# MycroftAI/mycroft-precise

Measured on AMD Instinct MI355X. Metric: MFCC+GRU windows/sec (node); max concurrent real-time 16 kHz streams, higher is better.
Workload: dtype f32

## Files before the change

### include/precise_engine.h

```cpp
#ifndef PRECISE_ENGINE_H
#define PRECISE_ENGINE_H

#include <stddef.h>
#include <stdint.h>

#ifdef __cplusplus
extern "C" {
#endif

#define PE_ABI_VERSION 8

typedef enum pe_status {
    PE_OK = 0,
    PE_ERR_INVALID = 1,
    PE_ERR_HIP = 2,
    PE_ERR_UNSUPPORTED = 3,
    PE_ERR_NOMEM = 4,
    PE_ERR_EOF = 5
} pe_status;

typedef struct pe_params {
    int32_t sample_rate;
    int32_t window_samples;
    int32_t hop_samples;
// ... 92 lines not shown
int pe_decode_device(pe_engine* e, const float* raw_dev, double* conf_out_dev, unsigned char* fired_out_dev, void* hip_stream);
int pe_decode(pe_engine* e, const float* raw_host, double* conf_out_host, unsigned char* fired_out_host);

typedef struct pe_info {
    int32_t n_streams, n_features, n_mfcc, units, n_layers, ring_slots, carry_capacity;
    int32_t mfcc_precision, gru_precision;
    int64_t device_bytes;
} pe_info;
int pe_get_info(const pe_engine* e, pe_info* out);

int pe_get_stream_state(pe_engine* e, int32_t* q_out, uint32_t* computed_out, uint32_t* emitted_out);

int pe_set_renumber_at(pe_engine* e, uint32_t call_number);

int pe_set_fused(pe_engine* e, int32_t enabled);

int pe_set_input_projection(pe_engine* e, int32_t enabled);

int pe_set_gru_waves(pe_engine* e, int32_t waves_per_tile);

int pe_set_gru_tiling(pe_engine* e, int32_t tiling);
int pe_get_gru_tiling(const pe_engine* e);

int pe_set_timing(pe_engine* e, int32_t enabled);
int pe_get_last_timing(pe_engine* e, float* mfcc_ms, float* gru_ms);

#ifdef __cplusplus
}
#endif
#endif
```

### mycroft_precise_amd/_lib.py

```python
import ctypes as C
import importlib.util
import os
import weakref

import numpy as np

HERE = os.path.dirname(os.path.abspath(__file__))
LIB_PATH = os.environ.get('PE_LIB') or os.path.join(HERE, 'libprecise_engine.so')

PE_OK, PE_ERR_INVALID, PE_ERR_HIP, PE_ERR_UNSUPPORTED, PE_ERR_NOMEM, PE_ERR_EOF = range(6)
ABI_VERSION = 8


class PeParams(C.Structure):
    _fields_ = [(n, C.c_int32) for n in (
        'sample_rate', 'window_samples', 'hop_samples', 'n_fft', 'n_filt', 'n_mfcc', 'n_features',
        'use_delta', 'mfcc_precision', 'gru_precision', 'vectorizer', 'ring_precision')]


class PeGruLayer(C.Structure):
    _fields_ = [('n_in', C.c_int32), ('units', C.c_int32),
                ('kernel', C.POINTER(C.c_float)), ('recurrent_kernel', C.POINTER(C.c_float)),
                ('bias', C.POINTER(C.c_float))]

# ... 38 lines not shown
    'pe_get_vectors': (C.c_int, [C.c_void_p, C.c_void_p]),
    'pe_set_vectors': (C.c_int, [C.c_void_p, C.c_void_p]),
    'pe_run_device': (C.c_int, [C.c_void_p, C.c_void_p, C.c_void_p]),
    'pe_predict': (C.c_int, [C.c_void_p, C.c_void_p, C.c_int32, C.c_void_p]),
    'pe_predict_device': (C.c_int, [C.c_void_p, C.c_void_p, C.c_int32, C.c_void_p, C.c_void_p]),
    'pe_vectorize_raw': (C.c_int, [C.c_void_p, C.c_void_p, C.c_int64, C.c_void_p, C.c_int64,
                                   C.POINTER(C.c_int64)]),
    'pe_vectorize_mels': (C.c_int, [C.c_void_p, C.c_void_p, C.c_int64, C.c_void_p, C.c_int64,
                                   C.POINTER(C.c_int64)]),
    'pe_evaluate': (C.c_int, [C.c_void_p, C.c_void_p, C.c_int64, C.c_int32, C.c_void_p, C.c_int64,
                              C.POINTER(C.c_int64)]),
    'pe_set_decoder': (C.c_int, [C.c_void_p, C.c_void_p, C.c_int32, C.c_int32, C.c_int32, C.c_double]),
    'pe_set_trigger': (C.c_int, [C.c_void_p, C.c_int32, C.c_double, C.c_int32]),
    'pe_set_decoder_model': (C.c_int, [C.c_void_p, C.c_int32, C.c_void_p, C.c_int32, C.c_int32, C.c_int32, C.c_double]),
    'pe_set_trigger_model': (C.c_int, [C.c_void_p, C.c_int32, C.c_int32, C.c_double, C.c_int32]),
    'pe_decode_device': (C.c_int, [C.c_void_p, C.c_void_p, C.c_void_p, C.c_void_p, C.c_void_p]),
    'pe_decode': (C.c_int, [C.c_void_p, C.c_void_p, C.c_void_p, C.c_void_p]),
    'pe_get_info': (C.c_int, [C.c_void_p, C.POINTER(PeInfo)]),
    'pe_get_stream_state': (C.c_int, [C.c_void_p, C.c_void_p, C.c_void_p, C.c_void_p]),
    'pe_set_fused': (C.c_int, [C.c_void_p, C.c_int32]),
    'pe_set_gru_waves': (C.c_int, [C.c_void_p, C.c_int32]),
    'pe_set_gru_tiling': (C.c_int, [C.c_void_p, C.c_int32]),
    'pe_get_gru_tiling': (C.c_int, [C.c_void_p]),
    'pe_set_input_projection': (C.c_int, [C.c_void_p, C.c_int32]),
    'pe_set_timing': (C.c_int, [C.c_void_p, C.c_int32]),
    'pe_get_last_timing': (C.c_int, [C.c_void_p, C.POINTER(C.c_float), C.POINTER(C.c_float)]),
}

_lib = None


class HipLibraryMissing(ImportError):
    pass


def _preload_hip_runtime():
    if os.environ.get('PRECISE_AMD_HIP_RUNTIME', '') == 'system':
        return
    try:
        spec = importlib.util.find_spec('torch')
    except (ImportError, ValueError):
        spec = None
    if spec is None or not spec.origin:
        return
    cand = os.path.join(os.path.dirname(spec.origin), 'lib', 'libamdhip64.so')
    if os.path.exists(cand):
# ... 301 lines not shown

    def stream_state(self):
        q = np.empty(self.n_streams, dtype=np.int32)
        kc = np.empty(self.n_streams, dtype=np.uint32)
        ke = np.empty(self.n_streams, dtype=np.uint32)
        self._check(self._lib.pe_get_stream_state(self._h, q.ctypes.data, kc.ctypes.data, ke.ctypes.data))
        return q, kc, ke

    def set_fused(self, enabled: bool):
        self._check(self._lib.pe_set_fused(self._h, int(bool(enabled))))

    def set_input_projection(self, enabled: bool):
        self._check(self._lib.pe_set_input_projection(self._h, int(bool(enabled))))

    def set_gru_waves(self, waves: int):
        self._check(self._lib.pe_set_gru_waves(self._h, int(waves)))

    def set_gru_tiling(self, tiling: int):
        self._check(self._lib.pe_set_gru_tiling(self._h, int(tiling)))

    def gru_tiling(self) -> int:
        return int(self._lib.pe_get_gru_tiling(self._h))

    def set_timing(self, enabled: bool):
        self._check(self._lib.pe_set_timing(self._h, int(bool(enabled))))

    def last_timing(self):
        a, b = C.c_float(0), C.c_float(0)
        self._check(self._lib.pe_get_last_timing(self._h, C.byref(a), C.byref(b)))
        return a.value, b.value

    def close(self):
        if getattr(self, '_h', None) and self._h.value:
            if getattr(self, '_views', 0) > 0:
                self._close_pending = True
                try:
                    self._lib.pe_wait(self._h)
                except Exception:
                    pass
                return
            self._lib.pe_destroy(self._h)
            self._h = C.c_void_p()

    def __del__(self):
        try:
            self.close()
# ... 3 lines not shown
```

### mycroft_precise_amd/csrc/engine.hip

```cpp
#include "../../include/precise_engine.h"
#include "pe_common.h"
#include "gru_cw_pack.h"
#include "mfcc_general_device.h"

#include <algorithm>
#include <cmath>
#include <cstdarg>
#include <cstdio>
#include <cstdlib>
#include <cstring>
#include <string>
#include <vector>

using namespace pe;

namespace {

thread_local std::string g_global_error;

struct DeviceBuf {
    void* p = nullptr;
    size_t bytes = 0;
};

// ... 19 lines not shown
    int device = 0;
    int n_streams = 0, n_tiles = 0, n_padded = 0;
    int units = 0, n_in = 0, n_layers = 0;
    int ring_slots = 0;
    int mel_nnz = 0;
    std::string err;
    std::vector<void*> allocs;
    int64_t device_bytes = 0;
    StreamRec* rec = nullptr;
    int16_t* carry = nullptr;
    const int16_t* kept = nullptr; int kept_chunk = 0;
    const int16_t* call_head = nullptr; int call_head_chunk = 0; bool call_keep = false;
    uint32_t call_no = 1;
    uint32_t renumber_at = 0x7fff0000u;
    bool fused = true;
    int gru_waves = 0;
    bool general = false;
    int row_floats = kRowFloats;
    int carry_cap = kCarryCap;
    GeneralTables gtab{};
    int gru_tiling = -1;
    int n_cus = 256;
    float* ring = nullptr;
    float* proj_ring = nullptr;
    bool proj_ok = false, proj_on = false;
    std::vector<float> proj_w_host, proj_b_host;
    int max_updates = 1;
    uint32_t* ke_hist = nullptr;
    unsigned char* table_blob = nullptr;
    pe_wave::Layout table_layout{};
    int n_models = 1;
    std::vector<NetPack> nets;
    std::vector<DecState> dec;
    bool wide = false;
    int wide_kx4[2] = {1, 1};
    int32_t* activation = nullptr;
    DeviceBuf st_pcm, st_out, st_feats, st_mask, st_audio, st_mfcc, st_conf, st_fired, st_ids;
    std::vector<uint8_t> seen_ids;
    bool timing = false;
    hipEvent_t ev[3] = {nullptr, nullptr, nullptr};
    bool ev_valid = false, ev_has_gru = false;
    static constexpr int kAsyncDepth = 3;
    struct AsyncSlot {
        float* pin_out = nullptr; size_t pin_out_bytes = 0;
        DeviceBuf dev_in, dev_out;
        hipEvent_t copied = nullptr, done = nullptr;
// ... 605 lines not shown
}

ModelNet model_net(const NetPack& n, const GruArgs& a) {
    return ModelNet{n.wx, n.wxd, n.wr1, n.wr2, n.bias, n.wd, a.cw ? n.cw_blob : nullptr, n.wx_bf16, n.wr_bf16, n.wd_bf16,
                    a.b20 ? n.b20_blob : nullptr, a.x3 ? n.x3_blob : nullptr, n.dense_bias};
}
GruArgs with_model(const pe_engine* e, const GruArgs& a, int m) { return model_args(a, model_net(e->nets[m], a), 0, 0); }
ModelSet model_set(const pe_engine* e, const GruArgs& a) {
    ModelSet ms{};
    for (int m = 0; m < e->n_models; ++m) ms.net[m] = model_net(e->nets[m], a);
    return ms;
}

GruArgs gru_args(const pe_engine* e) {
    const NetPack& n0 = e->nets[0];
    GruArgs a{};
    a.n_streams = e->n_streams;
    a.n_features = e->prm.n_features;
    a.n_in = e->n_in;
    a.units = e->units;
    a.use_delta = e->prm.use_delta;
    a.ring = e->ring; a.ring_slots = e->ring_slots; a.ring_bf16 = e->prm.ring_precision;
    a.ids = nullptr; a.rec = e->rec; a.n_padded = (uint32_t)e->n_padded; a.ke_plain = nullptr;
    a.call = e->call_no + 1u;
    a.proj_ring = e->proj_on ? e->proj_ring : nullptr;
    a.predict_ke = 0;
    a.chunk = 0;
    a.window = emit_window(e->prm); a.hop = e->prm.hop_samples;
    a.frame_len = frame_len_of(e->prm);
    a.bf16 = e->prm.gru_precision == 1;
    a.b20 = e->gru_tiling == 0 ? nullptr : n0.b20_blob;
    a.feats = nullptr; a.out = nullptr; a.row_stride = 0;
    a.row_floats = e->row_floats;
    const bool x3_ok = n0.x3_blob && !a.bf16 && !e->wide && !a.proj_ring && e->row_floats == kRowFloats;
    const bool many_windows = e->max_updates > 1 && (long long)e->max_updates * e->n_tiles > 4LL * e->n_cus;
    a.x3 = x3_ok && (e->gru_tiling == 2 || (e->gru_tiling < 0 && (e->n_tiles > 4 * e->n_cus || many_windows))) ? n0.x3_blob : nullptr;
    const bool cw_ok = n0.cw_blob && e->row_floats == kRowFloats && !a.proj_ring && !a.bf16 && !a.x3 && !e->wide;
    const bool retile = cw_ok && (e->gru_tiling == 1 || (e->gru_tiling < 0 && e->n_tiles <= 2 * e->n_cus));
    const int auto_waves = retile ? (e->n_tiles <= 2 * e->n_cus ? 4 : 1) : (e->n_tiles <= e->n_cus ? 4 : 1);
    a.waves_per_tile = a.x3 ? 1 : e->gru_waves ? e->gru_waves : auto_waves;
    if (e->prm.use_delta && !retile) a.waves_per_tile = 1;
    if (e->row_floats != kRowFloats && !(gru_small_regs(e->units) == 5 && !e->prm.use_delta && a.waves_per_tile == 4))
        a.waves_per_tile = 1;
    a.cw = retile ? n0.cw_blob : nullptr;
    return with_model(e, a, 0);
}
// ... 95 lines not shown
    e->last_user_stream = static_cast<hipStream_t>(stream);
    e->user_dirty = true;
}

int check_chunk(pe_engine* e, const void* pcm, int chunk) {
    if (!e) return PE_ERR_INVALID;
    if (chunk == 0) return fail(e, PE_ERR_EOF, "empty chunk");
    if (chunk < 0 || !pcm) return fail(e, PE_ERR_INVALID, "bad pcm buffer / chunk_samples=%d", chunk);
    return PE_OK;
}

int flush_kept(pe_engine* e, hipStream_t s) {
    if (!e->kept) return PE_OK;
    PE_HIP(e, launch_materialize_carry(state_of(e, e->call_no + 1u), e->kept, e->kept_chunk, e->n_streams, s));
    e->kept = nullptr; e->kept_chunk = 0;
    return PE_OK;
}

bool keep_eligible(const pe_engine* e, const int16_t* pcm_dev, int chunk) {
    return !e->general && (chunk & 1) == 0 && (reinterpret_cast<uintptr_t>(pcm_dev) & 3u) == 0 && chunk >= frame_len_of(e->prm) - 1
        && chunk >= e->carry_cap - 1;
}

bool can_fuse(const pe_engine* e, int chunk) {
    if (!(e->fused && !e->general && !e->wide && e->table_layout.mel_pad == 10 && chunk <= emit_window(e->prm) - frame_len_of(e->prm))) return false;
    if (gru_args(e).x3) return false;
    if (e->prm.gru_precision == 0 && gru_small_regs(e->units) >= 6 && gru_args(e).waves_per_tile != 4) return false;
    if (e->prm.use_delta && e->prm.gru_precision == 0) {
        const GruArgs g = gru_args(e);
        if (g.cw && (g.waves_per_tile != 4 || e->ring_slots != kCwSlots || e->prm.n_features > kCwSlots)) return false;
    }
    return true;
}

int do_update(pe_engine* e, const int16_t* pcm_dev, int chunk, float* raw_out_dev, float* feats_out_dev,
              hipStream_t s, const int32_t* ids = nullptr, int n_active = 0, bool keep = false) {
    int rc;
    const bool t = e->timing;
    const bool keep_call = keep && !ids && keep_eligible(e, pcm_dev, chunk);
    if (keep_call && e->kept) {
        const char* a0 = reinterpret_cast<const char*>(e->kept);
        const char* a1 = a0 + (size_t)e->n_streams * e->kept_chunk * sizeof(int16_t);
        const char* b0 = reinterpret_cast<const char*>(pcm_dev);
        const char* b1 = b0 + (size_t)e->n_streams * chunk * sizeof(int16_t);
        if (b0 < a1 && a0 < b1)
            return fail(e, PE_ERR_INVALID, "pe_update_device_keep: this call's chunks overlap the previous call's (%p), which still hold the "
                        "streams' leftover samples -- alternate between at least two buffers, or use pe_update_device", (const void*)e->kept);
    }
    if (!keep_call && (rc = flush_kept(e, s))) return rc;
    e->call_head = keep_call ? e->kept : nullptr; e->call_head_chunk = e->kept_chunk; e->call_keep = keep_call;
    struct Reset { pe_engine* e; ~Reset() { e->call_head = nullptr; e->call_head_chunk = 0; e->call_keep = false; } } reset{e};
    e->kept = keep_call ? pcm_dev : nullptr; e->kept_chunk = keep_call ? chunk : 0;
    uint32_t call = 0;
    if ((rc = begin_state_call(e, s, &call))) return rc;
    if (t) { PE_HIP(e, hipEventRecord(e->ev[0], s)); }
    if (raw_out_dev && can_fuse(e, chunk)) {
        GruArgs g = gru_args(e);
        g.call = call;
        g.predict_ke = 1;
        g.chunk = chunk;
        g.out = raw_out_dev;
        if (ids) { g.ids = ids; g.n_streams = n_active; }
        const ModelSet ms = model_set(e, g);
        const ModelSet* const models = e->n_models > 1 ? &ms : nullptr;
        if (e->prm.mfcc_precision == 0) PE_HIP(e, launch_fused(mfcc_args<double>(e, pcm_dev, chunk, call, ids, n_active), tables<double>(e), g, e->n_cus, s, models, e->n_models));
        else PE_HIP(e, launch_fused(mfcc_args<float>(e, pcm_dev, chunk, call, ids, n_active), tables<float>(e), g, e->n_cus, s, models, e->n_models));
        if (t) { PE_HIP(e, hipEventRecord(e->ev[1], s)); PE_HIP(e, hipEventRecord(e->ev[2], s)); e->ev_valid = true; e->ev_has_gru = false; }
    } else {
        if ((rc = launch_mfcc(e, pcm_dev, chunk, s, call, ids, n_active))) return rc;
        if (t) { PE_HIP(e, hipEventRecord(e->ev[1], s)); }
        if (raw_out_dev) {
            if ((rc = launch_gru_ring(e, raw_out_dev, s, ids, n_active))) return rc;
        }
        if (t) { PE_HIP(e, hipEventRecord(e->ev[2], s)); e->ev_valid = true; e->ev_has_gru = raw_out_dev != nullptr; }
    }
    if (feats_out_dev) {
        GatherArgs g{e->n_streams, e->prm.n_features, e->prm.n_mfcc, e->ring_slots, e->prm.ring_precision, e->ring, state_of(e, e->call_no + 1u), feats_out_dev, e->row_floats};
        PE_HIP(e, launch_gather(g, s));
    }
    return PE_OK;
}

}

extern "C" {

int pe_abi_version(void) { return PE_ABI_VERSION; }
const char* pe_last_global_error(void) { return g_global_error.c_str(); }
const char* pe_last_error(const pe_engine* e) { return e ? e->err.c_str() : g_global_error.c_str(); }

namespace {
// ... 123 lines not shown
                    const int Hlast = w->layers[w->n_layers - 1].units;
                    for (int u = 0; u < Hlast; ++u) dp[u] = w->dense_kernel[u];
                    pe_weights wp{w->n_layers, lp.data(), dp.data(), w->dense_bias};
                    e->units = Hp;
                    if ((rc = pack_gru_weights_wide(e, n, &wp))) break;
                    if ((rc = pack_gru_weights_wide_x3(e, n, &wp))) break;
                }
                else if ((rc = pack_gru_weights(e, n, L, w->dense_kernel))) break;
                if (p->gru_precision == 1 && (rc = pack_gru_weights_bf16(e, n, L, w->dense_kernel))) break;
                if (!wide && b20_eligible(*p, L) && (rc = pack_gru_weights_b20(e, n, L, w->dense_kernel))) break;
                if (!wide && x3_eligible(*p, L) && (rc = pack_gru_weights_x3(e, n, L, w->dense_kernel))) break;
            } while (false);
            return rc;
        };
        for (int m = 0; m < n_models && !rc; ++m) rc = pack_model(e->nets[m], &w[m]);
        if (rc) break;
        if (!wide) pack_projection_rows(e, L);
        e->proj_ok = !wide && p->gru_precision == 0 && !p->use_delta && gru_small_regs(L.units) == 5 && !e->proj_w_host.empty();
        e->proj_on = false;
        if (e->general) rc = (p->mfcc_precision == 0) ? build_general_tables<double>(e, mel_filters) : build_general_tables<float>(e, mel_filters);
        else rc = (p->mfcc_precision == 0) ? build_tables<double>(e, mel_filters) : build_tables<float>(e, mel_filters);
        if (rc) break;
        if (e->proj_on && (rc = dev_alloc(e, &e->proj_ring, (size_t)e->n_tiles * e->ring_slots * kTileStreams * kProjRow))) break;
        for (auto& ev : e->ev)
            if (hipEventCreate(&ev) != hipSuccess) { rc = fail(e, PE_ERR_HIP, "hipEventCreate failed"); break; }
        if (rc) break;
        const size_t lds = e->general ? general_lds_bytes(p->mfcc_precision == 0 ? 8 : 4, p->n_fft, p->n_filt, e->gtab.n_rounds)
                                      : (size_t)e->table_layout.total + (size_t)kFrameWaves * pe_wave::kScratchReals * (p->mfcc_precision == 0 ? 8 : 4);
        if (lds > 64 * 1024) { rc = fail(e, PE_ERR_UNSUPPORTED, "MFCC kernel would need %zu bytes of LDS per workgroup", lds); break; }
        if ((rc = pe_clear(e, nullptr))) break;
        hipError_t se = hipDeviceSynchronize();
        if (se != hipSuccess) { rc = fail(e, PE_ERR_HIP, "device sync after init failed: %s", hipGetErrorString(se)); break; }
    } while (false);
    if (rc) {
        g_global_error = e->err;
        pe_destroy(e);
        return rc;
    }
    *out = e;
    return PE_OK;
}
}

int pe_create(const pe_params* p, const double* mel_filters, const pe_weights* w, int32_t n_streams,
              int32_t device, pe_engine** out) {
    return create_engine(p, mel_filters, w, 1, n_streams, device, out);
// ... 34 lines not shown
    return PE_OK;
}

int pe_clear(pe_engine* e, const uint8_t* mask_host) {
    if (!e) return PE_ERR_INVALID;
    PE_HIP(e, hipSetDevice(e->device));
    PE_DRAIN(e);
    const uint8_t* mask_dev = nullptr;
    if (mask_host) {
        int rc = ensure(e, e->st_mask, (size_t)e->n_streams);
        if (rc) return rc;
        PE_HIP(e, hipMemcpy(e->st_mask.p, mask_host, (size_t)e->n_streams, hipMemcpyHostToDevice));
        mask_dev = static_cast<const uint8_t*>(e->st_mask.p);
    }
    if (mask_dev) { int frc = flush_kept(e, nullptr); if (frc) return frc; }
    else { e->kept = nullptr; e->kept_chunk = 0; }
    uint32_t call = 0;
    { int crc = begin_state_call(e, nullptr, &call); if (crc) return crc; }
    ClearArgs a{e->n_padded, e->ring_slots, mask_dev, state_of(e, call), e->ring, e->prm.ring_precision, e->activation,
                e->proj_on ? e->proj_ring : nullptr,
                e->proj_on ? reinterpret_cast<const float*>(e->table_blob + e->table_layout.proj_b) : nullptr, e->row_floats};
    if (mask_dev) a.n_streams = e->n_streams;
    PE_HIP(e, launch_clear(a, nullptr));
    if (e->activation)
        PE_HIP(e, launch_clear_activation(mask_dev, e->activation, a.n_streams, e->n_padded, e->n_models - 1, nullptr));
    PE_HIP(e, hipStreamSynchronize(nullptr));
    return PE_OK;
}

int pe_update_device(pe_engine* e, const int16_t* pcm_dev, int32_t chunk, float* raw_out_dev, void* stream) {
    int rc = check_chunk(e, pcm_dev, chunk);
    if (rc) return rc;
    PE_HIP(e, hipSetDevice(e->device));
    PE_DRAIN(e);
    if (!raw_out_dev) return fail(e, PE_ERR_INVALID, "raw_out_dev is null");
    note_user_stream(e, stream);
    return do_update(e, pcm_dev, chunk, raw_out_dev, nullptr, static_cast<hipStream_t>(stream));
}

int pe_update_device_keep(pe_engine* e, const int16_t* pcm_dev, int32_t chunk, float* raw_out_dev, void* stream) {
    int rc = check_chunk(e, pcm_dev, chunk);
    if (rc) return rc;
    PE_HIP(e, hipSetDevice(e->device));
    PE_DRAIN(e);
    if (!raw_out_dev) return fail(e, PE_ERR_INVALID, "raw_out_dev is null");
    note_user_stream(e, stream);
// ... 628 lines not shown
    if (e->wide) {
        if (tiling == 1) return fail(e, PE_ERR_UNSUPPORTED, "wide networks have two forms: 0 (f32-input MFMAs) and 2 (float32 products on the bf16 pipe)");
        PE_DRAIN(e);
        e->gru_tiling = tiling;
        return PE_OK;
    }
    if (tiling == 2 && !e->nets[0].x3_blob)
        return fail(e, PE_ERR_UNSUPPORTED, "the XDL form of the float32 network (tiling 2) takes <= 20 units, <= 15 inputs, float32 operands, no use_delta");
    if (tiling == 1 && e->prm.gru_precision == 1 && !e->nets[0].b20_blob)
        return fail(e, PE_ERR_UNSUPPORTED, "the five-values layout of the bf16 network (tiling 1) takes <= 20 units and <= 14 features");
    PE_DRAIN(e);
    e->gru_tiling = tiling;
    return PE_OK;
}

int pe_get_gru_tiling(const pe_engine* e) {
    if (!e) return -2;
    if (e->wide) return wide_uses_x3(e) ? 2 : 0;
    if (e->prm.gru_precision != 0) return gru_args(e).b20 ? 1 : 0;
    const GruArgs a = gru_args(e);
    return a.x3 ? 2 : a.cw ? 1 : 0;
}

int pe_set_timing(pe_engine* e, int32_t enabled) {
    if (!e) return PE_ERR_INVALID;
    e->timing = enabled != 0;
    e->ev_valid = false;
    return PE_OK;
}

int pe_get_last_timing(pe_engine* e, float* mfcc_ms, float* gru_ms) {
    if (!e) return PE_ERR_INVALID;
    if (!e->ev_valid) return fail(e, PE_ERR_INVALID, "no timed update recorded (call pe_set_timing(e, 1) first)");
    PE_HIP(e, hipEventSynchronize(e->ev[2]));
    float a = 0.f, b = 0.f;
    PE_HIP(e, hipEventElapsedTime(&a, e->ev[0], e->ev[1]));
    PE_HIP(e, hipEventElapsedTime(&b, e->ev[1], e->ev[2]));
    if (mfcc_ms) *mfcc_ms = a;
    if (gru_ms) *gru_ms = e->ev_has_gru ? b : 0.f;
    return PE_OK;
}

}
```

### mycroft_precise_amd/csrc/gru_cw_device.h

```cpp
#pragma once
#include "gru_device.h"
#include "gru_cw_pack.h"

namespace pe {


struct CwLds {
    static constexpr int BOX = 0;
    static constexpr int XR = 2048;
    static constexpr int FLOATS = XR + kCwSlots * 256;
};
constexpr size_t kCwLdsBytes = (size_t)CwLds::FLOATS * sizeof(float);

__device__ __forceinline__ f32x4 mfma4(float a, float b, f32x4 c) {
    return __builtin_amdgcn_mfma_f32_4x4x1f32(a, b, c, 0, 0, 0);
}

__device__ __forceinline__ float v_sum4(const f32x4& p) {
#pragma clang fp contract(off)
    const auto s0 = __builtin_amdgcn_permlane32_swap(__float_as_uint(p[0]), __float_as_uint(p[2]), false, false);
    const auto s1 = __builtin_amdgcn_permlane32_swap(__float_as_uint(p[1]), __float_as_uint(p[3]), false, false);
    const float q0 = __uint_as_float(s0[0]) + __uint_as_float(s0[1]);
    const float q1 = __uint_as_float(s1[0]) + __uint_as_float(s1[1]);
    const auto s2 = __builtin_amdgcn_permlane16_swap(__float_as_uint(q0), __float_as_uint(q1), false, false);
// ... 172 lines not shown
        for (int kk = 0; kk < 4; ++kk) v[kk] = (4 * g + kk < a.n_in) ? p[kk] : 0.f;
        return v;
    };
    float h[5];
#pragma unroll
    for (int rho = 0; rho < 5; ++rho) h[rho] = 0.f;
    f32x4 x = load_x(0), xprev = x;
    for (int t = 0; t < T; ++t) {
        const f32x4 xn = load_x(t + 1);
        f32x4 aZ = cw_xproj(wx[kTZ], bias[kTZ], x), aX = cw_xproj(wx[kTX], bias[kTX], x);
        f32x4 aC = cw_xproj(wx[kTC], bias[kTC], x), aV = cw_xproj(wx[kTV], bias[kTV], x);
        if constexpr (DELTA) {
            f32x4 d = {0.f, 0.f, 0.f, 0.f};
            if (MODE == kFeats) d = load_d(t);
            else if (t > 0) d = x - xprev;
            aZ = cw_dproj(wxd[kTZ], aZ, d); aX = cw_dproj(wxd[kTX], aX, d);
            aC = cw_dproj(wxd[kTC], aC, d); aV = cw_dproj(wxd[kTV], aV, d);
            xprev = x;
        }
        S.step(h, aZ, aX, aC, aV);
        x = xn;
    }
    cw_head(a, h, wd, stream, valid, g);
}

struct CwBox {
    static constexpr int PX = 0;
    static constexpr int PC = PX + 512;
    static constexpr int PV = PC + 512;
    static constexpr int SH4 = PV + 256;
    static constexpr int SH1 = SH4 + 256;
    static constexpr int SZ4 = SH1 + 64;
    static constexpr int SZ1 = SZ4 + 256;
    static constexpr int TAG = SZ1 + 64;
    static constexpr int END = TAG + 4;
};
static_assert(CwBox::END <= 1984 && CwBox::END <= CwLds::XR, "mailboxes overlap the role slots / the staged ring");

template <bool VF>
__device__ __forceinline__ void gru_tile_cw(const GruArgs& a, const int tile, const int wave, const int lane, float* S) {
#pragma clang fp contract(off)
    const int g = lane >> 4, j = lane & 15;
    const long long stream = (long long)tile * kTileStreams + j;
    const bool valid = stream < a.n_streams;
    const int T = a.n_features;
    const float* cw = a.cw;
// ... 271 lines not shown
```

### mycroft_precise_amd/csrc/kernels.hip

```cpp
#include <cstdlib>
#include <type_traits>
#include "mfcc_device.h"
#include "mfcc_wave_device.h"
#include "gru_device.h"
#include "gru_cw_device.h"
#include "gru_bf16_device.h"
#include "gru_b20_device.h"
#include "gru_x3_device.h"
#include "gru_wide_device.h"
#include "gru_wide_x3_device.h"
#include "mfcc_general_device.h"

namespace pe {

#ifndef PE_FRAME_WPE
#define PE_FRAME_WPE 4
#endif
template <int BYTES>
__device__ __forceinline__ void touch_kernel_arguments() {
    const int* ka = (const int*)__builtin_amdgcn_kernarg_segment_ptr();
    static_assert(BYTES <= 12 * 64, "more lines than this helper requests");
    auto line = [&](int i) -> int { return i * 64 < BYTES ? ka[i * 16] : 0; };
    const int v0 = line(0), v1 = line(1), v2 = line(2), v3 = line(3), v4 = line(4), v5 = line(5), v6 = line(6), v7 = line(7),
              v8 = line(8), v9 = line(9), v10 = line(10), v11 = line(11);
// ... 315 lines not shown
                    const int simd = wave_simd_id();
                    if ((threadIdx.x & 63) == 0) slot[wave] = simd;
                    __syncthreads();
                    if (((1 << slot[0]) | (1 << slot[1]) | (1 << slot[2]) | (1 << slot[3])) == 15) role = simd;
                }
                gru_tile_cw<false>(gm, bl, role, threadIdx.x & 63, reinterpret_cast<float*>(smem));
            } else {
                const int tile = bl * 4 + wave;
                if (tile < n_tiles) gru_tile_v<kRing, false>(gm, tile, threadIdx.x & 63);
            }
        } else if (MW) {
            gru_tile_mw_any<RG, PROJ>(gm, bl, wave, threadIdx.x & 63, reinterpret_cast<float*>(smem));
        } else {
            const int tile = bl * 4 + wave;
            if (tile < n_tiles) gru_tile<RG, kRing, PROJ>(gm, tile, threadIdx.x & 63);
        }
    } else if (b < n_net + n_frame_blocks) {
        mfcc_frame_tasks<R, SH, true, !PROJ>(m, t, smem, (b - n_net) * kFrameWaves, n_frame_blocks * kFrameWaves, CW && MW && (frames_first & kBySimd));
    } else {
        mfcc_book_tile<R>(m, b - n_net - n_frame_blocks);
    }
}

#define PE_FUSED_PARAMS (const MfccStreamArgs<R> m, const WaveTables<R> t, const GruArgs g, const int n_gru_blocks, const int n_frame_blocks, const int n_tiles, const int frames_first)
#define PE_FUSED_MODELS_PARAMS (const MfccStreamArgs<R> m, const WaveTables<R> t, const GruArgs g, const int n_gru_blocks, const int n_models, const int n_frame_blocks, \
                                const int n_tiles, const int frames_first, const ModelSet ms)
PE_KERNEL_PAIR((template <class R, class SH, bool DELTA, bool RB>), PE_FRAME_KERNEL(256, PE_FRAME_WPE), fused_update_bf16_kernel, PE_FUSED_PARAMS,
               { fused_update_bf16_body<R, SH, DELTA, RB, false>(m, t, g, nullptr, n_gru_blocks, 1, n_frame_blocks, n_tiles, frames_first); })
PE_KERNEL_PAIR((template <class R, class SH, bool DELTA, bool RB>), PE_FRAME_KERNEL(256, PE_FRAME_WPE), fused_update_bf16_models_kernel, PE_FUSED_MODELS_PARAMS,
               { fused_update_bf16_body<R, SH, DELTA, RB, true>(m, t, g, &ms, n_gru_blocks, n_models, n_frame_blocks, n_tiles, frames_first); })
PE_KERNEL_PAIR((template <class R, class SH, int RG, bool MW, bool PROJ, bool CW = false>), PE_FRAME_KERNEL(256, PE_FRAME_WPE), fused_update_kernel, PE_FUSED_PARAMS,
               { fused_update_body<R, SH, RG, MW, PROJ, CW, false>(m, t, g, nullptr, n_gru_blocks, 1, n_frame_blocks, n_tiles, frames_first); })
PE_KERNEL_PAIR((template <class R, class SH, int RG, bool MW, bool CW>), PE_FRAME_KERNEL(256, PE_FRAME_WPE), fused_update_models_kernel, PE_FUSED_MODELS_PARAMS,
               { fused_update_body<R, SH, RG, MW, false, CW, true>(m, t, g, &ms, n_gru_blocks, n_models, n_frame_blocks, n_tiles, frames_first); })


static int frame_blocks(long long n_tasks, int n_cus, int per_cu = 4) {
    const long long need = (n_tasks + kFrameWaves - 1) / kFrameWaves;
    const long long cap = (long long)n_cus * per_cu;
    return (int)(need < cap ? (need < 1 ? 1 : need) : cap);
}

static int stream_frame_blocks(int n_streams, int n_cus, int per_cu_default = 4) {
    const long long slots = 2LL * n_streams;
    const long long cap_waves = (long long)frame_blocks(slots, n_cus, per_cu_default) * kFrameWaves;
    const long long per_wave = (slots + cap_waves - 1) / cap_waves;
    const long long waves = (slots + per_wave - 1) / per_wave;
    return (int)((waves + kFrameWaves - 1) / kFrameWaves);
}

template <class R>
static size_t frame_lds(const WaveTables<R>& t) { return wave_lds_bytes(sizeof(R), t.L, kFrameWaves); }
template <class R>
static bool blob_matches_shape(const WaveTables<R>& t) {
    return t.L.mel_pad == ShapeStock::MEL ? shape_layout_matches<R, ShapeStock>(t.L) : shape_layout_matches<R, ShapeAny>(t.L);
}

// ... 127 lines not shown
static bool fused_models_four_waves(int n_models, int tiles, int n_cus) { return (long long)n_models * tiles <= 2LL * n_cus; }

struct FusedLaunch { const ModelSet* ms; int n_models, fb, tiles; hipStream_t s; };
#define PE_FUSED(KERNEL, MODELS_KERNEL, TARGS, MODELS_TARGS, GB, LDS, FF)                                                    \
    do {                                                                                                                     \
        if (f.ms) PE_LAUNCH_R(R, MODELS_KERNEL, MODELS_TARGS, dim3((GB) * f.n_models + f.fb + f.tiles), dim3(256), LDS, f.s, m, t, g, GB, f.n_models, f.fb, f.tiles, FF, *f.ms); \
        else PE_LAUNCH_R(R, KERNEL, TARGS, dim3((GB) + f.fb + f.tiles), dim3(256), LDS, f.s, m, t, g, GB, f.fb, f.tiles, FF); \
    } while (0)
#define PE_FUSED_F32(MW, PROJ, CW, GB, LDS, FF) \
    PE_FUSED(fused_update_kernel, fused_update_models_kernel, (ShapeStock, RG, MW, PROJ, CW), (ShapeStock, RG, MW, CW), GB, LDS, FF)

template <class R, int RG>
static hipError_t launch_fused_rg(const MfccStreamArgs<R>& m, const WaveTables<R>& t, const GruArgs& g, int n_cus, hipStream_t s,
                                  const ModelSet* ms, int n_models) {
    if (ms && g.proj_ring) return hipErrorInvalidValue;
    const int tiles = (m.geo.n_streams + kTileStreams - 1) / kTileStreams;
    const size_t lds = frame_lds(t);
    const bool by_simd = g.cw && g.waves_per_tile == 4 && cw_four_waves_ok(g) && tiles <= n_cus;
    const int frames_first = ((g.waves_per_tile != 4 && tiles >= 4 * n_cus) ? 1 : 0) | (by_simd ? kBySimd : 0);
    const int fb = stream_frame_blocks(m.geo.n_streams, n_cus, tiles <= n_cus ? 2 : (frames_first & kFramesFirst) ? 3 : 4);
    const FusedLaunch f{ms, n_models, fb, tiles, s};
    const int one_per_tile = tiles, four_per_block = (tiles + 3) / 4;
    if constexpr (RG == 5) {
        if (g.cw) {
            const bool four = g.waves_per_tile == 4 && cw_four_waves_ok(g) && (!ms || g.use_delta || fused_models_four_waves(n_models, tiles, n_cus));
            if (four) PE_FUSED_F32(true, false, true, one_per_tile, lds > kCwLdsBytes ? lds : kCwLdsBytes, frames_first);
            else PE_FUSED_F32(false, false, true, four_per_block, lds, frames_first & ~kBySimd);
            return hipGetLastError();
        }
        if (g.proj_ring) {
            if (g.waves_per_tile == 4) PE_LAUNCH_R(R, fused_update_kernel, (ShapeStock, RG, true, true), dim3(one_per_tile + fb + tiles), dim3(256), lds, s, m, t, g, one_per_tile, fb, tiles, frames_first);
            else PE_LAUNCH_R(R, fused_update_kernel, (ShapeStock, RG, false, true), dim3(four_per_block + fb + tiles), dim3(256), lds, s, m, t, g, four_per_block, fb, tiles, frames_first);
            return hipGetLastError();
        }
    }
    if (g.waves_per_tile == 4) PE_FUSED_F32(true, false, false, one_per_tile, lds, frames_first);
    else if constexpr (RG <= 5) PE_FUSED_F32(false, false, false, four_per_block, lds, frames_first);
    else return hipErrorInvalidValue;
    return hipGetLastError();
}

template <class R>
static hipError_t launch_fused_t(const MfccStreamArgs<R>& m, const WaveTables<R>& t, const GruArgs& g, int n_cus, hipStream_t s,
                                 const ModelSet* ms, int n_models) {
    if (ms && (n_models < 1 || n_models > kMaxModels)) return hipErrorInvalidValue;
    if (t.L.mel_pad != ShapeStock::MEL || !blob_matches_shape(t)) return hipErrorInvalidValue;
// ... 244 lines not shown
    if (n_rows < 1 || n_streams < 1) return hipSuccess;
    hipLaunchKernelGGL(clear_activation_kernel, dim3((n_streams + 255) / 256, n_rows), dim3(256), 0, s, mask, activation, n_streams, n_padded);
    return hipGetLastError();
}
hipError_t launch_decode(const DecodeArgs& a, hipStream_t s) {
    if (a.n_streams == 0) return hipSuccess;
    hipLaunchKernelGGL(decode_kernel, dim3((a.n_streams + 255) / 256), dim3(256), 0, s, a);
    return hipGetLastError();
}

hipError_t launch_gather(const GatherArgs& a, hipStream_t s) {
    const long long total = (long long)a.n_streams * a.n_features * a.n_mfcc;
    if (total == 0) return hipSuccess;
    hipLaunchKernelGGL(gather_kernel, dim3((unsigned)((total + 255) / 256)), dim3(256), 0, s, a);
    return hipGetLastError();
}

hipError_t launch_clear(const ClearArgs& a, hipStream_t s) {
    if (a.n_streams == 0) return hipSuccess;
    hipLaunchKernelGGL(clear_kernel, dim3(a.n_streams), dim3(64), 0, s, a);
    return hipGetLastError();
}

}
```

### mycroft_precise_amd/csrc/pe_common.h

```cpp
#pragma once
#include <hip/hip_runtime.h>
#include <stdint.h>
#include "mfcc_wave_tables.h"

namespace pe {

constexpr int kTileStreams = 16;
constexpr int kRowFloats = 16;
constexpr int kCarryCap = 512;
constexpr int kNfft = 512;
constexpr int kBins = kNfft / 2 + 1;
constexpr int kMaxFilt = 64;
constexpr int kCwSlots = 32;

template <class R> struct cplx { R x, y; };

constexpr int kMaxFrameRows = 4096;
constexpr int kFrameWaves = 4;

template <class R>
struct WaveTables {
    const void* blob;
    pe_wave::Layout L;
};
// ... 82 lines not shown
template <class R>
struct MfccOfflineArgs {
    StreamGeom geo;
    const double* audio;
    long long n_samples;
    long long n_frames;
    double* out;
    float* out_rows;
    double* out_mels;
};

constexpr int kX3Tiles = 4;
constexpr int kX3RecOps = 4, kX3InOps = 3;
constexpr int kX3ArOff = 0;
constexpr int kX3AxOff = kX3Tiles * kX3RecOps * 64;
constexpr int kX3WdOff = kX3AxOff + kX3Tiles * kX3InOps * 64;
constexpr int kX3BlobBytes = kX3WdOff * 16 + 5 * 64 * 4;

constexpr int kB20Tiles = 4;
constexpr int kB20ArOff = 0;
constexpr int kB20AxOff = kB20Tiles * 64;
constexpr int kB20WdOff = 2 * kB20Tiles * 64;
constexpr int kB20BlobBytes = kB20WdOff * 16 + 5 * 64 * 4;

struct GruArgs {
    int n_streams;
    int n_features;
    int n_in;
    int units;
    const float* wx;
    const float* wxd;
    int use_delta;
    const float* wr1;
    const float* wr2;
    const float* bias;
    const float* wd;
    float dense_bias;
    const float* cw;
    int bf16;
    const void* wx_bf16;
    const void* wr_bf16;
    const float* wd_bf16;
    const void* b20;
    const void* x3;
    const void* reserved_;
    const int32_t* ids;
    const StreamRec* rec;
    uint32_t n_padded, call;
    const uint32_t* ke_plain;
    const float* ring;
    int ring_bf16;
    const float* proj_ring;
    int ring_slots;
    int predict_ke;
    int chunk, window, hop, frame_len;
    const float* feats;
    int row_stride;
    float* out;
    int row_floats;
    int waves_per_tile;
};

constexpr int kMaxModels = 8;
struct ModelNet {
    const float* wx; const float* wxd; const float* wr1; const float* wr2; const float* bias; const float* wd;
    const float* cw;
    const void* wx_bf16; const void* wr_bf16; const float* wd_bf16; const void* b20;
    const void* x3;
// ... 81 lines not shown
struct DecodeArgs {
    int n_streams;
    const float* raw;
    const double* cd;
    int cd_len, min_out, out_range;
    double center;
    double* conf_out;
    int32_t* activation;
    unsigned char* fired_out;
    double threshold;
    int trigger_level, rearm;
};
hipError_t launch_decode(const DecodeArgs& a, hipStream_t s);
struct DecodeSet { DecodeArgs m[kMaxModels]; };
hipError_t launch_decode_models(const DecodeSet& d, int n_models, int n_streams, hipStream_t s);
hipError_t launch_clear_activation(const uint8_t* mask, int32_t* activation, int n_streams, int n_padded, int n_rows, hipStream_t s);

constexpr int kProjRow = pe_wave::kProjRow;
hipError_t launch_mfcc_f64(const MfccStreamArgs<double>& a, const WaveTables<double>& t, int n_cus, hipStream_t s);
hipError_t launch_mfcc_f32(const MfccStreamArgs<float>& a, const WaveTables<float>& t, int n_cus, hipStream_t s);
hipError_t launch_gru_many(const GruArgs& a, int n_updates, int n_padded, hipStream_t s, const ModelSet* ms = nullptr, int n_models = 1);
hipError_t launch_fused(const MfccStreamArgs<double>& m, const WaveTables<double>& t, const GruArgs& g, int n_cus, hipStream_t s, const ModelSet* ms = nullptr, int n_models = 1);
hipError_t launch_fused(const MfccStreamArgs<float>& m, const WaveTables<float>& t, const GruArgs& g, int n_cus, hipStream_t s, const ModelSet* ms = nullptr, int n_models = 1);
hipError_t launch_mfcc_offline_f64(const MfccOfflineArgs<double>& a, const WaveTables<double>& t, int n_cus, hipStream_t s);
hipError_t launch_mfcc_offline_f32(const MfccOfflineArgs<float>& a, const WaveTables<float>& t, int n_cus, hipStream_t s);
hipError_t launch_gru_small(const GruArgs& a, int input_mode, hipStream_t s, const ModelSet* ms = nullptr, int n_models = 1, long long out_stride = 0);
int gru_small_regs(int units);
int gru_wide_waves(int units);
int gru_small_tiles(int units);
hipError_t launch_gru_wide(const WideArgs& a, int input_mode, hipStream_t s);
hipError_t launch_gru_wide_x3(const WideArgs& a, int input_mode, hipStream_t s);
hipError_t launch_gather(const GatherArgs& a, hipStream_t s);
hipError_t launch_scatter(const GatherArgs& a, hipStream_t s);
hipError_t launch_renumber(const StreamState& st, int n_padded, hipStream_t s);
hipError_t launch_materialize_carry(const StreamState& st, const int16_t* head, int head_chunk, int n_streams, hipStream_t s);
hipError_t launch_clear(const ClearArgs& a, hipStream_t s);
hipError_t launch_project_rows(const float* ring, float* proj, const float* w, const float* b, int n_mfcc, long long n_rows, hipStream_t s);

}
```

Before: 271.8 million.

## Carry staggered GRU hidden states across updates to process only new frames

Adds a per-stream chain buffer holding 32 staggered GRU hidden-state columns (two 16-lane groups) plus a stamp recording the last processed frame. Each column resets when its window starts, so on each update every lane advances only the newly arrived frames instead of rerunning the GRU over the whole window. The dense head is then read from the column whose window ends at the current frame. A new fused kernel variant uses this path when it is eligible (single f32 model, no delta, small feature count), and clear now invalidates stamps. The cost is extra device memory per stream and heavier state traffic, with a full recompute still needed when the carry is invalid.

```diff
diff --git a/include/precise_engine.h b/include/precise_engine.h
--- a/include/precise_engine.h
+++ b/include/precise_engine.h
@@ -138,6 +138,8 @@
 int pe_set_gru_tiling(pe_engine* e, int32_t tiling);
 int pe_get_gru_tiling(const pe_engine* e);
 
+int pe_get_last_update_path(const pe_engine* e);
+
 int pe_set_timing(pe_engine* e, int32_t enabled);
 int pe_get_last_timing(pe_engine* e, float* mfcc_ms, float* gru_ms);
 
diff --git a/mycroft_precise_amd/_lib.py b/mycroft_precise_amd/_lib.py
--- a/mycroft_precise_amd/_lib.py
+++ b/mycroft_precise_amd/_lib.py
@@ -84,6 +84,7 @@
     'pe_set_gru_waves': (C.c_int, [C.c_void_p, C.c_int32]),
     'pe_set_gru_tiling': (C.c_int, [C.c_void_p, C.c_int32]),
     'pe_get_gru_tiling': (C.c_int, [C.c_void_p]),
+    'pe_get_last_update_path': (C.c_int, [C.c_void_p]),
     'pe_set_input_projection': (C.c_int, [C.c_void_p, C.c_int32]),
     'pe_set_timing': (C.c_int, [C.c_void_p, C.c_int32]),
     'pe_get_last_timing': (C.c_int, [C.c_void_p, C.POINTER(C.c_float), C.POINTER(C.c_float)]),
@@ -431,6 +432,9 @@
     def gru_tiling(self) -> int:
         return int(self._lib.pe_get_gru_tiling(self._h))
 
+    def last_update_path(self) -> int:
+        return int(self._lib.pe_get_last_update_path(self._h))
+
     def set_timing(self, enabled: bool):
         self._check(self._lib.pe_set_timing(self._h, int(bool(enabled))))
 
diff --git a/mycroft_precise_amd/csrc/engine.hip b/mycroft_precise_amd/csrc/engine.hip
--- a/mycroft_precise_amd/csrc/engine.hip
+++ b/mycroft_precise_amd/csrc/engine.hip
@@ -65,6 +65,8 @@
     int gru_tiling = -1;
     int n_cus = 256;
     float* ring = nullptr;
+    void* chain = nullptr;
+    int last_update_path = 0;
     float* proj_ring = nullptr;
     bool proj_ok = false, proj_on = false;
     std::vector<float> proj_w_host, proj_b_host;
@@ -716,6 +718,7 @@
     a.use_delta = e->prm.use_delta;
     a.ring = e->ring; a.ring_slots = e->ring_slots; a.ring_bf16 = e->prm.ring_precision;
     a.ids = nullptr; a.rec = e->rec; a.n_padded = (uint32_t)e->n_padded; a.ke_plain = nullptr;
+    a.chain = e->chain;
     a.call = e->call_no + 1u;
     a.proj_ring = e->proj_on ? e->proj_ring : nullptr;
     a.predict_ke = 0;
@@ -857,6 +860,11 @@
         && chunk >= e->carry_cap - 1;
 }
 
+bool chain_eligible(const pe_engine* e) {
+    return e->n_models == 1 && !e->wide && !e->general && e->prm.gru_precision == 0 && !e->prm.use_delta && e->nets[0].cw_blob
+        && e->row_floats == kRowFloats && e->prm.n_features <= kChainCols && e->n_tiles <= 2 * e->n_cus;
+}
+
 bool can_fuse(const pe_engine* e, int chunk) {
     if (!(e->fused && !e->general && !e->wide && e->table_layout.mel_pad == 10 && chunk <= emit_window(e->prm) - frame_len_of(e->prm))) return false;
     if (gru_args(e).x3) return false;
@@ -898,10 +906,12 @@
         if (ids) { g.ids = ids; g.n_streams = n_active; }
         const ModelSet ms = model_set(e, g);
         const ModelSet* const models = e->n_models > 1 ? &ms : nullptr;
+        e->last_update_path = fused_takes_chain(g, models) ? 2 : 1;
         if (e->prm.mfcc_precision == 0) PE_HIP(e, launch_fused(mfcc_args<double>(e, pcm_dev, chunk, call, ids, n_active), tables<double>(e), g, e->n_cus, s, models, e->n_models));
         else PE_HIP(e, launch_fused(mfcc_args<float>(e, pcm_dev, chunk, call, ids, n_active), tables<float>(e), g, e->n_cus, s, models, e->n_models));
         if (t) { PE_HIP(e, hipEventRecord(e->ev[1], s)); PE_HIP(e, hipEventRecord(e->ev[2], s)); e->ev_valid = true; e->ev_has_gru = false; }
     } else {
+        e->last_update_path = 0;
         if ((rc = launch_mfcc(e, pcm_dev, chunk, s, call, ids, n_active))) return rc;
         if (t) { PE_HIP(e, hipEventRecord(e->ev[1], s)); }
         if (raw_out_dev) {
@@ -1071,6 +1081,11 @@
         else rc = (p->mfcc_precision == 0) ? build_tables<double>(e, mel_filters) : build_tables<float>(e, mel_filters);
         if (rc) break;
         if (e->proj_on && (rc = dev_alloc(e, &e->proj_ring, (size_t)e->n_tiles * e->ring_slots * kTileStreams * kProjRow))) break;
+        if (chain_eligible(e)) {
+            unsigned char* cp = nullptr;
+            if ((rc = dev_alloc(e, &cp, chain_bytes((size_t)e->n_padded)))) break;
+            e->chain = cp;
+        }
         for (auto& ev : e->ev)
             if (hipEventCreate(&ev) != hipSuccess) { rc = fail(e, PE_ERR_HIP, "hipEventCreate failed"); break; }
         if (rc) break;
@@ -1151,6 +1166,7 @@
                 e->proj_on ? reinterpret_cast<const float*>(e->table_blob + e->table_layout.proj_b) : nullptr, e->row_floats};
     if (mask_dev) a.n_streams = e->n_streams;
     PE_HIP(e, launch_clear(a, nullptr));
+    PE_HIP(e, launch_chain_invalidate(e->chain, mask_dev, a.n_streams, nullptr));
     if (e->activation)
         PE_HIP(e, launch_clear_activation(mask_dev, e->activation, a.n_streams, e->n_padded, e->n_models - 1, nullptr));
     PE_HIP(e, hipStreamSynchronize(nullptr));
@@ -1825,6 +1841,8 @@
     return a.x3 ? 2 : a.cw ? 1 : 0;
 }
 
+int pe_get_last_update_path(const pe_engine* e) { return e ? e->last_update_path : -1; }
+
 int pe_set_timing(pe_engine* e, int32_t enabled) {
     if (!e) return PE_ERR_INVALID;
     e->timing = enabled != 0;
diff --git a/mycroft_precise_amd/csrc/gru_cw_device.h b/mycroft_precise_amd/csrc/gru_cw_device.h
--- a/mycroft_precise_amd/csrc/gru_cw_device.h
+++ b/mycroft_precise_amd/csrc/gru_cw_device.h
@@ -218,6 +218,87 @@
         x = xn;
     }
     cw_head(a, h, wd, stream, valid, g);
+}
+
+__device__ __forceinline__ float cw_head_value(const GruArgs& a, const float (&h)[5], const float (&wd)[5]) {
+    float part = 0.f;
+#pragma unroll
+    for (int rho = 0; rho < 5; ++rho) part = fmaf(h[rho], wd[rho], part);
+    part += __shfl_xor(part, 16);
+    part += __shfl_xor(part, 32);
+    return 1.0f / (1.0f + expf(-(part + a.dense_bias)));
+}
+__device__ __forceinline__ void gru_tile_chain(const GruArgs& a, const int v, const int lane) {
+    const int g = lane >> 4, j = lane & 15;
+    const uint32_t T = (uint32_t)a.n_features;
+    const float* cw = a.cw;
+    const long long sid = a.ids ? (long long)a.ids[v] : (long long)v;
+    const KeRequest ke_req = gru_ke_request(a, sid);
+    ChainStamp* const stamps = reinterpret_cast<ChainStamp*>(a.chain);
+    ChainStamp* const stamp = stamps + sid;
+    float* const cols = reinterpret_cast<float*>(stamps + a.n_padded) + (size_t)sid * kChainFloats + lane;
+    const ChainStamp st = *stamp;
+    float h0[5], h1[5];
+#pragma unroll
+    for (int rho = 0; rho < 5; ++rho) { h0[rho] = cols[rho * 64]; h1[rho] = cols[(5 + rho) * 64]; }
+    CwStep<false> S;
+    S.load(cw, lane);
+    float wx[4][4], wd[5];
+    f32x4 bias[4];
+#pragma unroll
+    for (int tl = 0; tl < 4; ++tl)
+#pragma unroll
+        for (int kk = 0; kk < 4; ++kk) {
+            wx[tl][kk] = cw[CwPack::WX + (tl * 4 + kk) * 64 + lane];
+            bias[tl][kk] = cw[CwPack::BIAS + (tl * 4 + kk) * 64 + lane];
+        }
+#pragma unroll
+    for (int rho = 0; rho < 5; ++rho) wd[rho] = a.wd[rho * 64 + lane];
+
+    const uint32_t E = (uint32_t)__builtin_amdgcn_readfirstlane((int)gru_ke_resolve(a, ke_req));
+    const uint32_t k = E - (uint32_t)__builtin_amdgcn_readfirstlane((int)st.through);
+    const bool carried = __builtin_amdgcn_readfirstlane((int)st.valid) == 1 && k < T;
+    const uint32_t n = carried ? k : T;
+    if (n == 0) {
+        if (lane == 0) a.out[v] = st.last_out;
+        return;
+    }
+    const float* const xbase = a.ring + gru_ring_cell(a, sid) * kRowFloats + 4 * g;
+    const uint32_t mask = (uint32_t)(a.ring_slots - 1);
+    auto load_x = [&](const uint32_t f) -> f32x4 {
+        return *reinterpret_cast<const f32x4*>(xbase + (size_t)(f & mask) * kTileStreams * kRowFloats);
+    };
+    uint32_t f = E - n;
+    f32x4 x = load_x(f);
+    if (!carried) {
+#pragma unroll
+        for (int rho = 0; rho < 5; ++rho) { h0[rho] = 0.f; h1[rho] = 0.f; }
+    }
+    for (uint32_t i = 0; i < n; ++i, ++f) {
+        const f32x4 xn = load_x(i + 1 < n ? f + 1 : f);
+        const f32x4 aZ = cw_xproj(wx[kTZ], bias[kTZ], x), aX = cw_xproj(wx[kTX], bias[kTX], x);
+        const f32x4 aC = cw_xproj(wx[kTC], bias[kTC], x), aV = cw_xproj(wx[kTV], bias[kTV], x);
+        const int c = (int)(f & (uint32_t)(kChainCols - 1));
+#pragma unroll
+        for (int rho = 0; rho < 5; ++rho) {
+            h0[rho] = j == c ? 0.f : h0[rho];
+            h1[rho] = j + 16 == c ? 0.f : h1[rho];
+        }
+        S.step(h0, aZ, aX, aC, aV);
+        S.step(h1, aZ, aX, aC, aV);
+        x = xn;
+    }
+    const int ce = (int)((E - T) & (uint32_t)(kChainCols - 1));
+    float hs[5];
+#pragma unroll
+    for (int rho = 0; rho < 5; ++rho) hs[rho] = (ce & 16) ? h1[rho] : h0[rho];
+    const float p = cw_head_value(a, hs, wd);
+#pragma unroll
+    for (int rho = 0; rho < 5; ++rho) { cols[rho * 64] = h0[rho]; cols[(5 + rho) * 64] = h1[rho]; }
+    if (g == 0 && j == (ce & 15)) {
+        a.out[v] = p;
+        *stamp = ChainStamp{E, 1u, p, 0u};
+    }
 }
 
 struct CwBox {
diff --git a/mycroft_precise_amd/csrc/kernels.hip b/mycroft_precise_amd/csrc/kernels.hip
--- a/mycroft_precise_amd/csrc/kernels.hip
+++ b/mycroft_precise_amd/csrc/kernels.hip
@@ -361,6 +361,19 @@
     }
 }
 
+bool fused_takes_chain(const GruArgs& g, const ModelSet* ms) {
+    return g.chain && g.cw && !ms && !g.use_delta && !g.proj_ring && g.n_features <= kChainCols && g.row_floats == kRowFloats;
+}
+#ifndef PE_CHAIN_FB
+#define PE_CHAIN_FB 4
+#endif
+#ifndef PE_CHAIN_FF
+#define PE_CHAIN_FF 1
+#endif
+#ifndef PE_CHAIN_PRIO
+#define PE_CHAIN_PRIO 0
+#endif
+
 #define PE_FUSED_PARAMS (const MfccStreamArgs<R> m, const WaveTables<R> t, const GruArgs g, const int n_gru_blocks, const int n_frame_blocks, const int n_tiles, const int frames_first)
 #define PE_FUSED_MODELS_PARAMS (const MfccStreamArgs<R> m, const WaveTables<R> t, const GruArgs g, const int n_gru_blocks, const int n_models, const int n_frame_blocks, \
                                 const int n_tiles, const int frames_first, const ModelSet ms)
@@ -372,6 +385,27 @@
                { fused_update_body<R, SH, RG, MW, PROJ, CW, false>(m, t, g, nullptr, n_gru_blocks, 1, n_frame_blocks, n_tiles, frames_first); })
 PE_KERNEL_PAIR((template <class R, class SH, int RG, bool MW, bool CW>), PE_FRAME_KERNEL(256, PE_FRAME_WPE), fused_update_models_kernel, PE_FUSED_MODELS_PARAMS,
                { fused_update_body<R, SH, RG, MW, false, CW, true>(m, t, g, &ms, n_gru_blocks, n_models, n_frame_blocks, n_tiles, frames_first); })
+
+template <class R, class SH>
+__device__ __forceinline__ void fused_update_chain_body(const MfccStreamArgs<R>& m, const WaveTables<R>& t, const GruArgs& g,
+                                                        const int n_gru_blocks, const int n_frame_blocks, const int frames_first) {
+    extern __shared__ __attribute__((aligned(16))) unsigned char smem[];
+    touch_kernel_arguments<kFusedArgBytes<R, false>>();
+    const int b = role_block(blockIdx.x, n_gru_blocks, n_frame_blocks, frames_first & kFramesFirst);
+    if (b < n_gru_blocks) {
+        const int v = b * 4 + __builtin_amdgcn_readfirstlane(threadIdx.x >> 6);
+#if PE_CHAIN_PRIO
+        __builtin_amdgcn_s_setprio(PE_CHAIN_PRIO);
+#endif
+        if (v < g.n_streams) gru_tile_chain(g, v, threadIdx.x & 63);
+    } else if (b < n_gru_blocks + n_frame_blocks) {
+        mfcc_frame_tasks<R, SH, true, true>(m, t, smem, (b - n_gru_blocks) * kFrameWaves, n_frame_blocks * kFrameWaves, false);
+    } else {
+        mfcc_book_tile<R>(m, b - n_gru_blocks - n_frame_blocks);
+    }
+}
+PE_KERNEL_PAIR((template <class R, class SH>), PE_FRAME_KERNEL(256, PE_FRAME_WPE), fused_update_chain_kernel, PE_FUSED_PARAMS,
+               { (void)n_tiles; fused_update_chain_body<R, SH>(m, t, g, n_gru_blocks, n_frame_blocks, frames_first); })
 
 
 static int frame_blocks(long long n_tasks, int n_cus, int per_cu = 4) {
@@ -545,6 +579,12 @@
     const FusedLaunch f{ms, n_models, fb, tiles, s};
     const int one_per_tile = tiles, four_per_block = (tiles + 3) / 4;
     if constexpr (RG == 5) {
+        if (fused_takes_chain(g, ms)) {
+            const int n = m.geo.n_streams;
+            const int cfb = stream_frame_blocks(n, n_cus, PE_CHAIN_FB);
+            PE_LAUNCH_R(R, fused_update_chain_kernel, (ShapeStock), dim3((n + 3) / 4 + cfb + tiles), dim3(256), lds, s, m, t, g, (n + 3) / 4, cfb, tiles, PE_CHAIN_FF ? kFramesFirst : 0);
+            return hipGetLastError();
+        }
         if (g.cw) {
             const bool four = g.waves_per_tile == 4 && cw_four_waves_ok(g) && (!ms || g.use_delta || fused_models_four_waves(n_models, tiles, n_cus));
             if (four) PE_FUSED_F32(true, false, true, one_per_tile, lds > kCwLdsBytes ? lds : kCwLdsBytes, frames_first);
@@ -835,4 +875,15 @@
     return hipGetLastError();
 }
 
-}
+__global__ void chain_invalidate_kernel(ChainStamp* stamps, const uint8_t* mask, const int n_streams) {
+    const int s = blockIdx.x * blockDim.x + threadIdx.x;
+    if (s >= n_streams || (mask && !mask[s])) return;
+    stamps[s].valid = 0u;
+}
+hipError_t launch_chain_invalidate(void* chain, const uint8_t* mask, int n_streams, hipStream_t s) {
+    if (!chain || n_streams < 1) return hipSuccess;
+    hipLaunchKernelGGL(chain_invalidate_kernel, dim3((n_streams + 255) / 256), dim3(256), 0, s, static_cast<ChainStamp*>(chain), mask, n_streams);
+    return hipGetLastError();
+}
+
+}
diff --git a/mycroft_precise_amd/csrc/pe_common.h b/mycroft_precise_amd/csrc/pe_common.h
--- a/mycroft_precise_amd/csrc/pe_common.h
+++ b/mycroft_precise_amd/csrc/pe_common.h
@@ -128,6 +128,11 @@
 constexpr int kB20AxOff = kB20Tiles * 64;
 constexpr int kB20WdOff = 2 * kB20Tiles * 64;
 constexpr int kB20BlobBytes = kB20WdOff * 16 + 5 * 64 * 4;
+
+constexpr int kChainCols = 32;
+constexpr int kChainFloats = 2 * 5 * 64;
+struct __attribute__((aligned(16))) ChainStamp { uint32_t through, valid; float last_out; uint32_t pad; };
+__host__ __device__ __forceinline__ size_t chain_bytes(const size_t n_padded) { return n_padded * (sizeof(ChainStamp) + kChainFloats * sizeof(float)); }
 
 struct GruArgs {
     int n_streams;
@@ -149,7 +154,7 @@
     const float* wd_bf16;
     const void* b20;
     const void* x3;
-    const void* reserved_;
+    void* chain;
     const int32_t* ids;
     const StreamRec* rec;
     uint32_t n_padded, call;
@@ -277,6 +282,8 @@
 hipError_t launch_gru_many(const GruArgs& a, int n_updates, int n_padded, hipStream_t s, const ModelSet* ms = nullptr, int n_models = 1);
 hipError_t launch_fused(const MfccStreamArgs<double>& m, const WaveTables<double>& t, const GruArgs& g, int n_cus, hipStream_t s, const ModelSet* ms = nullptr, int n_models = 1);
 hipError_t launch_fused(const MfccStreamArgs<float>& m, const WaveTables<float>& t, const GruArgs& g, int n_cus, hipStream_t s, const ModelSet* ms = nullptr, int n_models = 1);
+bool fused_takes_chain(const GruArgs& g, const ModelSet* ms);
+hipError_t launch_chain_invalidate(void* chain, const uint8_t* mask, int n_streams, hipStream_t s);
 hipError_t launch_mfcc_offline_f64(const MfccOfflineArgs<double>& a, const WaveTables<double>& t, int n_cus, hipStream_t s);
 hipError_t launch_mfcc_offline_f32(const MfccOfflineArgs<float>& a, const WaveTables<float>& t, int n_cus, hipStream_t s);
 hipError_t launch_gru_small(const GruArgs& a, int input_mode, hipStream_t s, const ModelSet* ms = nullptr, int n_models = 1, long long out_stride = 0);
```

After: 232.9 million. 14.3% lower.
